# MengLcool/RichSem

Hardware: AMD Instinct MI355X
Metric: training images/sec, RichSem R50 4-scale 1333x800 (MSDeformAttn hot path: 12 fwd + 12 bwd calls per step) (higher is better)
Workload: dtype f32; 1 GPU; configs[1]: R50 4-scale 800x1344 (S=22323), bs=2/GPU, M=8 D=32 L=P=4; per step 6x E(Lq=22323) + 6x Dd(Lq=1092), forward and backward, 12 distinct per-layer tensor sets; loc-init; loc=init, images_per_gpu=2, parallelism=dp1 (replicas, no collective)

## Files before the change

richsem_amd/csrc/msda_rps.h:

```cpp
#pragma once

#include <algorithm>
#include <atomic>
#include <vector>

#include "msda_common.h"

namespace msda {

constexpr int kRpsThreads = 768;
constexpr int kRpsWaves = kRpsThreads / 64;
constexpr int kRpsMaxPx = 312;
constexpr int kRpsMaxSide = 31;
constexpr int kRpsScanThreads = (kRpsMaxPx + 63) / 64 * 64, kRpsScanWaves = kRpsScanThreads / 64;
constexpr int kRpsPpq = (kRpsMaxPx + kRpsThreads / 4 - 1) / (kRpsThreads / 4);
constexpr int kRpsRpl = 2;
constexpr int kRpsChunk = kRpsRpl * kRpsThreads;
constexpr int kRpsSumStride = 36;
constexpr int kRpsSegShift = 3;
constexpr int kRpsMaxSegs = kRpsMaxPx + (kRpsChunk >> kRpsSegShift);
constexpr int kRpsMaxL = 4;
constexpr int kRpsMaxUnits = 448;
constexpr int kRpsD = 32;
constexpr int kRpsPad = 32;
constexpr int kRpsDummyWgs = 2048, kRpsDummyBytes = kRpsDummyWgs * 1024;
constexpr int kRpsMaxRuns = 320;
constexpr int kRpsRunSearch = 256;
static_assert(kRpsRunSearch < kRpsMaxRuns && 2 * kRpsRunSearch >= kRpsMaxRuns, "run search");
constexpr int kRpsQpBits = 19;
constexpr int kRpsPxBits = 9;
static_assert(kRpsMaxPx <= 1 << kRpsPxBits && kRpsQpBits + kRpsPxBits + 4 == 32, "record code: qp | base-grid index | corners");
static_assert(kRpsMaxPx <= kRpsMaxSide * kRpsMaxSide && kRpsScanThreads <= kRpsThreads && kRpsScanWaves * 4 <= 32, "tile grid");
static_assert(kRpsChunk < 1 << 16, "a list's length and a chunk's unit count share a 32-bit word in the scan; slot[] is 16 bits wide");

struct RpsLevel {
    int H, W, start;
    int TH, TW, nty, ntx;
    int bin0;
    int nslab;
    int atomic;
    float inv_TH, inv_TW;
};

struct alignas(16) RpsRec {
    unsigned code;
    float lh, lw, a;
};

struct RpsGeom {
    int N, S, M, Lq, L, P;
    int nunits, ppx;
    int bins_per_pair, nbins;
    RpsLevel lv[kRpsMaxL];
    unsigned units[kRpsMaxUnits];
    unsigned *ctr;
    unsigned long long *bin_state;
    uint2 *runs;
    int max_runs;
    int route_threads;
    unsigned entries_cap;
    struct RpsRec *entries;
    int lut_r[kRpsMaxL], lut_c[kRpsMaxL], lut_n;
    int seg_shift;
    float *dummy;
    unsigned long long *stamps;
};

struct alignas(16) RpsEnt {
    float lh;
    float hwa, lwa;
    unsigned row;
};

struct RpsLds {
    int item_slot[2];
    int wave_tot[16];
    int n_segs, pad[3];
    int uhist[32];
    uint2 runs[kRpsMaxRuns];
    unsigned long long stamp_last, stamp_acc[14];
    int offs[kRpsScanThreads + 4];
    unsigned seg[kRpsMaxSegs + 16];
    RpsEnt ent[kRpsChunk];
    unsigned short slot[kRpsChunk];
    alignas(16) double sum[kRpsMaxPx * kRpsSumStride];
    alignas(16) float vtile[kRpsMaxPx * kRpsD];
};
static_assert(sizeof(RpsLds) <= 160 * 1024, "rps: LDS budget");

__device__ __forceinline__ int rps_wave_scan(int v)
{
    v += __builtin_amdgcn_update_dpp(0, v, 0x111, 0xF, 0xF, true);
    v += __builtin_amdgcn_update_dpp(0, v, 0x112, 0xF, 0xF, true);
    v += __builtin_amdgcn_update_dpp(0, v, 0x114, 0xF, 0xF, true);
    v += __builtin_amdgcn_update_dpp(0, v, 0x118, 0xF, 0xF, true);
    v += __builtin_amdgcn_update_dpp(0, v, 0x142, 0xA, 0xF, false);
    v += __builtin_amdgcn_update_dpp(0, v, 0x143, 0xC, 0xF, false);
    return v;
}

#define RPS_STAMP(i)                                                                   \
    if (kStamps && g.stamps && threadIdx.x == 0) {                                     \
        const unsigned long long now_ = __builtin_amdgcn_s_memtime();                  \
        S->stamp_acc[i] += now_ - S->stamp_last;                                       \
        S->stamp_last = now_;                                                          \
    }

__device__ __forceinline__ unsigned rps_lut_row(const RpsLevel &v, int r)
{
    const int h_low = r - 1, br = max(h_low, 0);
    const int ty = (int)(((float)br + 0.5f) * v.inv_TH);
    const int R0 = ty * v.TH;
    const unsigned gr = (unsigned)(h_low - R0 + 1);
    const unsigned inr = (h_low >= 0 ? 1u : 0u) | (h_low + 1 < v.H ? 2u : 0u);
    return gr | inr << 6 | (unsigned)(ty * v.ntx * v.nslab) << 8;
}
__device__ __forceinline__ unsigned rps_lut_col(const RpsLevel &v, int c)
{
    const int w_low = c - 1, bc = max(w_low, 0);
    const int tx = (int)(((float)bc + 0.5f) * v.inv_TW);
    const int C0 = tx * v.TW, C1 = min(v.W, C0 + v.TW);
    const unsigned gc = (unsigned)(w_low - C0 + 1);
    const unsigned inc = (w_low >= 0 ? 1u : 0u) | (w_low + 1 < v.W ? 2u : 0u);
    const unsigned gw = (unsigned)(C1 - C0 + 1);
    return gc | inc << 6 | (unsigned)(tx * v.nslab) << 8 | gw << 17;
}

constexpr int kRpsRouteThreadsMax = 1024;
static_assert(kRpsMaxUnits <= 512, "route pass: one thread per bin of a pair");

template <int kRpsRouteThreads, int kL = 0, int kP = 0, bool kStamps = false>
__global__ __launch_bounds__(kRpsRouteThreads, 4) void rps_route_kernel(const float *__restrict__ loc, const float *__restrict__ aw,
                                                                     float *__restrict__ grad_value, float *__restrict__ grad_loc,
                                                                     float *__restrict__ grad_aw, const RpsGeom g)
{
    __shared__ unsigned hist[kRpsMaxUnits], base[512];
    __shared__ unsigned wtot[kRpsRouteThreads / kWave];
    __shared__ unsigned sink[kWave];
    extern __shared__ unsigned rps_lut[];
    const int tid = threadIdx.x, lane = tid & (kWave - 1), wave = tid / kWave;
    const int B = g.bins_per_pair;
    const int L = kL ? kL : g.L;
    {
        const int gtid = blockIdx.x * blockDim.x + tid, gsz = gridDim.x * blockDim.x;
        if (gtid < 8) g.ctr[gtid] = 0u;
        if (tid < kWave) sink[tid] = 0u;
        const int row4 = g.M * kRpsD / 4;
        for (int l = 0; l < L; ++l) {
            const RpsLevel &v = g.lv[l];
            for (int i = tid; i <= v.H; i += kRpsRouteThreads) rps_lut[g.lut_r[l] + i] = rps_lut_row(v, i);
            for (int i = tid; i <= v.W; i += kRpsRouteThreads) rps_lut[g.lut_c[l] + i] = rps_lut_col(v, i);
            if (!v.atomic) {
                const int nb = v.nty * v.W + v.ntx * v.H;
                for (int b = 0; b < g.N; ++b) {
                    float4 *dst = reinterpret_cast<float4 *>(grad_value) + (size_t)(b * g.S + v.start) * row4;
                    for (int i = gtid; i < nb * row4; i += gsz) {
                        const int k = i / row4, c = i - k * row4;
                        int px;
                        if (k < v.nty * v.W) {
                            const int ty = k / v.W;
                            px = ty * v.TH * v.W + (k - ty * v.W);
                        } else {
                            const int k2 = k - v.nty * v.W, tx = k2 / v.H;
                            px = (k2 - tx * v.H) * v.W + tx * v.TW;
                        }
                        dst[(size_t)px * row4 + c] = make_float4(0.f, 0.f, 0.f, 0.f);
                    }
                }
                continue;
            }
            const int n4 = v.H * v.W * row4;
            for (int b = 0; b < g.N; ++b) {
                float4 *dst = reinterpret_cast<float4 *>(grad_value) + (size_t)(b * g.S + v.start) * row4;
                for (int i = gtid; i < n4; i += gsz) dst[i] = make_float4(0.f, 0.f, 0.f, 0.f);
            }
        }
    }
    const int P = kP ? kP : g.P, LP = L * P;
    const int qpw = P <= 4 ? 16 : (P <= 8 ? 8 : (P <= 16 ? 4 : (P <= 32 ? 2 : 1)));
    const int ql = lane / P, pp = lane - ql * P;
    const int qpb = qpw * (kRpsRouteThreads / kWave);
    const int qblocks = (g.Lq + qpb - 1) / qpb;
    const int pairs = g.N * g.M;
    const int n_items = pairs * qblocks;
    const unsigned long long lt_mask = (1ull << lane) - 1ull;
    unsigned long long st_acc[8] = {0, 0, 0, 0, 0, 0, 0, 0}, st_last = kStamps && g.stamps ? __builtin_amdgcn_s_memtime() : 0ull;
#define RPS_RSTAMP(i)                                                  \
    if (kStamps && g.stamps) {                                         \
        const unsigned long long now_ = __builtin_amdgcn_s_memtime();  \
        st_acc[i] += now_ - st_last;                                   \
        st_last = now_;                                                \
    }
    float2 xy[kRpsMaxL];
    const int step_pair = (int)(gridDim.x % (unsigned)pairs), step_qb = (int)(gridDim.x / (unsigned)pairs);
    auto item_point = [&](int item_, int pair_, int qb_, bool &live_, int &q_) {
        const int b_ = pair_ / g.M, m_ = pair_ - b_ * g.M;
        q_ = qb_ * qpb + wave * qpw + ql;
        live_ = item_ < n_items && ql < qpw && pp < P && q_ < g.Lq;
        return (unsigned)(((b_ * g.Lq + (live_ ? q_ : 0)) * g.M + m_) * LP + min(pp, P - 1));
    };
    auto request_xy = [&](int item_, int pair_, int qb_) {
        bool live_;
        int q_;
        const unsigned pt0_ = item_point(item_, pair_, qb_, live_, q_);
#pragma unroll
        for (int l = 0; l < kRpsMaxL; ++l) xy[l] = *reinterpret_cast<const float2 *>(loc + 2u * (pt0_ + (unsigned)(min(l, L - 1) * P)));
    };
    int pair = (int)(blockIdx.x % (unsigned)pairs), qb = (int)(blockIdx.x / (unsigned)pairs);
    request_xy(blockIdx.x, pair, qb);
    unsigned long long p_old = 0ull;
    unsigned p_first = 0u, p_cnt = 0u;
    size_t p_gb = 0;
    for (int item = blockIdx.x; item < n_items; item += gridDim.x) {
        for (int i = tid; i < B; i += kRpsRouteThreads) hist[i] = 0u;
        bool live;
        int q;
        const unsigned pt0 = item_point(item, pair, qb, live, q);
        int n_pair = pair + step_pair, n_qb = qb + step_qb;
        if (n_pair >= pairs) {
            n_pair -= pairs;
            ++n_qb;
        }
        n_qb = min(n_qb, qblocks - 1);
        __syncthreads();
        RPS_RSTAMP(1)
        unsigned word[kRpsMaxL];
        unsigned inmap[kRpsMaxL];
        float lh[kRpsMaxL], lw[kRpsMaxL];
        unsigned re[kRpsMaxL], ce[kRpsMaxL];
        unsigned valid_m = 0u, asked_m = 0u, matched_m = 0u;
        unsigned dropped = 0u;
#pragma unroll
        for (int l = 0; l < kRpsMaxL; ++l) {
            lh[l] = lw[l] = 0.f;
            re[l] = ce[l] = 0u;
            if (l >= L) continue;
            const RpsLevel &v = g.lv[l];
            const float Hf = (float)v.H, Wf = (float)v.W;
            const float h_im = xy[l].y * Hf - 0.5f, w_im = xy[l].x * Wf - 0.5f;
            const bool valid = live && h_im > -1.f && w_im > -1.f && h_im < Hf && w_im < Wf;
            valid_m |= valid ? 1u << l : 0u;
            const float hf = floorf(h_im), wf = floorf(w_im);
            lh[l] = h_im - hf;
            lw[l] = w_im - wf;
            dropped |= live && !valid ? 1u << l : 0u;
            re[l] = rps_lut[g.lut_r[l] + (valid ? (int)hf + 1 : 0)];
            ce[l] = rps_lut[g.lut_c[l] + (valid ? (int)wf + 1 : 0)];
        }
        request_xy(item + (int)gridDim.x, n_pair, n_qb);
        float at[kRpsMaxL];
#pragma unroll
        for (int l = 0; l < kRpsMaxL; ++l) at[l] = aw[pt0 + (unsigned)(min(l, L - 1) * P)];
        int ob[kRpsMaxL], lead[kRpsMaxL], lb[kRpsMaxL];
        unsigned own_rank[kRpsMaxL], lt_cnt[kRpsMaxL], n_match[kRpsMaxL];
#pragma unroll
        for (int l = 0; l < kRpsMaxL; ++l) {
            ob[l] = -1;
            lead[l] = 0;
            lb[l] = -1;
            own_rank[l] = lt_cnt[l] = n_match[l] = 0u;
            inmap[l] = 0u;
            word[l] = ~0u;
            if (l >= L) continue;
            const RpsLevel &v = g.lv[l];
            const int ns = v.nslab;
            const int slab = ns > 1 ? uni(qb % ns) : 0;
            ob[l] = (valid_m >> l & 1u) ? v.bin0 + slab + (int)(re[l] >> 8) + (int)((ce[l] >> 8) & 511u) : -1;
            const unsigned inr = (re[l] >> 6) & 3u, inc = (ce[l] >> 6) & 3u;
            inmap[l] = ((inr & 1u) ? inc : 0u) | ((inr & 2u) ? inc << 2 : 0u);
            const unsigned long long vote = __ballot(ob[l] >= 0);
            const int ld = vote ? __ffsll((long long)vote) - 1 : 0;
            lb[l] = __builtin_amdgcn_readlane(ob[l], ld);
            const unsigned long long match = __ballot(ob[l] == lb[l]);
            lead[l] = ld;
            matched_m |= ob[l] == lb[l] && lb[l] >= 0 ? 1u << l : 0u;
            lt_cnt[l] = (unsigned)__popcll(match & lt_mask);
            n_match[l] = (unsigned)__popcll(match);
        }
#pragma unroll
        for (int l = 0; l < kRpsMaxL; ++l) {
            const bool is_lead = lane == lead[l] && lb[l] >= 0, other = ob[l] >= 0 && ob[l] != lb[l];
            const bool asked = is_lead || other;
            asked_m |= asked ? 1u << l : 0u;
            own_rank[l] = atomicAdd(asked ? &hist[is_lead ? lb[l] : ob[l]] : &sink[lane], is_lead ? n_match[l] : (other ? 1u : 0u));
        }
#pragma unroll
        for (int l = 0; l < kRpsMaxL; ++l) {
            if (l >= L) continue;
            const unsigned gr = re[l] & 31u, gc = ce[l] & 31u;
            if (!(asked_m >> l & 1u)) own_rank[l] = lt_cnt[l];
            if (ob[l] >= 0) word[l] = (unsigned)ob[l] | (gr * ((ce[l] >> 17) & 31u) + gc) << 23;
        }
        RPS_RSTAMP(2)
        __syncthreads();
        RPS_RSTAMP(3)
        const unsigned cnt = tid < B ? hist[tid] : 0u;
        const unsigned incl = (unsigned)rps_wave_scan((int)cnt);
        if (lane == kWave - 1) wtot[wave] = incl;
        __syncthreads();
        unsigned before = 0u;
#pragma unroll
        for (int w = 0; w < kRpsRouteThreads / kWave; ++w) before += w < wave ? wtot[w] : 0u;
        const unsigned first = (unsigned)item * (unsigned)(qpb * LP) + before + incl - cnt;
        if (cnt) base[tid] = first;
#pragma unroll
        for (int l = 0; l < kRpsMaxL; ++l) {
            if (l >= L) continue;
            unsigned r = own_rank[l];
            const unsigned rl = (unsigned)__builtin_amdgcn_readlane((int)r, lead[l]);
            if ((matched_m >> l & 1u) && lane != lead[l]) r += rl;
            if (word[l] != ~0u) word[l] |= r << 9;
        }
        __syncthreads();
        RPS_RSTAMP(4)
        const size_t gb = (size_t)pair * B + min(tid, B - 1);
        unsigned long long *const scratch64 = reinterpret_cast<unsigned long long *>(g.dummy + (size_t)(blockIdx.x & (kRpsDummyWgs - 1)) * 256) + lane;
        if (p_cnt) g.runs[p_gb * (size_t)g.max_runs + (size_t)min((unsigned)(p_old >> 32), (unsigned)g.max_runs - 1u)] = make_uint2(p_first, (unsigned)p_old);
        const unsigned long long old = atomicAdd(cnt ? g.bin_state + gb * (kRpsPad / 2) : scratch64, cnt ? (1ull << 32) | (unsigned long long)cnt : 0ull);
        const unsigned qp = (unsigned)((live ? q : 0) * P + pp);
        unsigned slot0[kRpsMaxL];
#pragma unroll
        for (int l = 0; l < kRpsMaxL; ++l) slot0[l] = base[word[l] & 511u];
        asm volatile("" : "+v"(at[0]), "+v"(at[1]), "+v"(at[2]), "+v"(at[3]));
#pragma unroll
        for (int l = 0; l < kRpsMaxL; ++l) {
            const unsigned w = word[l];
            if (w != ~0u) {
                const unsigned slot = min(slot0[l] + ((w >> 9) & 16383u), g.entries_cap - 1u);
                const unsigned code = qp | (w >> 23) << kRpsQpBits | inmap[l] << (kRpsQpBits + kRpsPxBits);
                g.entries[slot] = RpsRec{code, lh[l], lw[l], at[l]};
            }
        }
        if (__ballot(dropped != 0u)) {
#pragma unroll
            for (int l = 0; l < kRpsMaxL; ++l)
                if (dropped >> l & 1u) {
                    const unsigned pt = pt0 + (unsigned)(l * P);
                    grad_aw[pt] = 0.f;
                    *reinterpret_cast<float2 *>(grad_loc + 2u * pt) = make_float2(0.f, 0.f);
                }
        }
        RPS_RSTAMP(5)
        p_old = old;
        p_first = first;
        p_cnt = cnt;
        p_gb = gb;
        pair = n_pair;
        qb = n_qb;
        RPS_RSTAMP(6)
        __syncthreads();
        RPS_RSTAMP(7)
    }
    if (p_cnt) g.runs[p_gb * (size_t)g.max_runs + (size_t)min((unsigned)(p_old >> 32), (unsigned)g.max_runs - 1u)] = make_uint2(p_first, (unsigned)p_old);
    if (kStamps && g.stamps && tid == 0)
        for (int i = 0; i < 8; ++i) g.stamps[(size_t)(1024 + blockIdx.x) * 16 + i] = st_acc[i];
#undef RPS_RSTAMP
}

typedef float rps_v2f __attribute__((ext_vector_type(2)));
typedef float rps_v4f __attribute__((ext_vector_type(4)));

__device__ __forceinline__ float rps_quad_rotated_sum(float x0, float x1, float x2, float x3)
{
    const float ra = x0 + dpp_f<kDppXor1>(x1);
    const float rb = x2 + dpp_f<kDppXor1>(x3);
    return ra + dpp_f<kDppXor2>(rb);
}

template <typename TV>
struct RpsRow;
template <>
struct RpsRow<float> {
    float4 a, b;
    __device__ __forceinline__ void load(const float *base, unsigned off)
    {
        a = *reinterpret_cast<const float4 *>(reinterpret_cast<const char *>(base) + off);
        b = *reinterpret_cast<const float4 *>(reinterpret_cast<const char *>(base) + off + 64u);
    }
    __device__ __forceinline__ void unpack(rps_v2f (&gq)[4]) const
    {
        gq[0] = (rps_v2f){a.x, a.y}; gq[1] = (rps_v2f){a.z, a.w};
        gq[2] = (rps_v2f){b.x, b.y}; gq[3] = (rps_v2f){b.z, b.w};
    }
};
template <>
struct RpsRow<bf16_t> {
    uint2 a, b;
    __device__ __forceinline__ void load(const bf16_t *base, unsigned off)
    {
        a = *reinterpret_cast<const uint2 *>(reinterpret_cast<const char *>(base) + off);
        b = *reinterpret_cast<const uint2 *>(reinterpret_cast<const char *>(base) + off + 32u);
    }
    __device__ __forceinline__ void unpack(rps_v2f (&gq)[4]) const
    {
        gq[0] = (rps_v2f){__uint_as_float(a.x << 16), __uint_as_float(a.x & 0xFFFF0000u)};
        gq[1] = (rps_v2f){__uint_as_float(a.y << 16), __uint_as_float(a.y & 0xFFFF0000u)};
        gq[2] = (rps_v2f){__uint_as_float(b.x << 16), __uint_as_float(b.x & 0xFFFF0000u)};
        gq[3] = (rps_v2f){__uint_as_float(b.y << 16), __uint_as_float(b.y & 0xFFFF0000u)};
    }
};

template <bool P4, typename TV = float, bool kStamps = false>
__global__ __launch_bounds__(kRpsThreads, kRpsThreads / 256) void rps_tile_kernel(
    const TV *__restrict__ value, const TV *__restrict__ grad_out, TV *__restrict__ grad_value, float *__restrict__ grad_acc,
    float *__restrict__ grad_loc, float *__restrict__ grad_aw, const RpsGeom g)
{
    extern __shared__ __attribute__((aligned(16))) unsigned char smem[];
    RpsLds *S = reinterpret_cast<RpsLds *>(smem);

    const int tid = threadIdx.x, lane = tid & (kWave - 1), wave = tid / kWave;
    const int j4 = tid & 3, quad = tid >> 2;
    const int c_lo = 4 * j4, c_hi = 16 + 4 * j4;
    const float w_ys = (j4 & 2) ? 1.f : -1.f, w_yc = (j4 & 2) ? 0.f : 1.f;
    const unsigned w_xoff = (j4 & 1) ? 8u : 4u;
    const unsigned lane_row = (unsigned)(c_lo * sizeof(TV));
    const int P = P4 ? 4 : g.P;
    const int LP = g.L * P;
    const int row_elems = g.M * kRpsD;
    const int pairs = g.N * g.M;
    const int xq = blockIdx.x & (kXcds - 1);
    const int n_items = g.nunits * g.ppx;
    float *const dummy_w = g.dummy + (size_t)(blockIdx.x & (kRpsDummyWgs - 1)) * 256;
    if (kStamps && g.stamps && tid == 0) {
        for (int i = 0; i < 14; ++i) S->stamp_acc[i] = 0;
        S->stamp_last = __builtin_amdgcn_s_memtime();
    }
    struct Item {
        bool live;
        int l, b, m, H, W, R0, R1, C0, C1, gw, npx;
    };
    auto item_geom = [&](int id) {
        Item it;
        const unsigned unit = (unsigned)uni((int)g.units[min(id, n_items - 1) / g.ppx]);
        const int pr = xq + kXcds * (min(id, n_items - 1) % g.ppx);
        const int pair = min(pr, pairs - 1);
        it.live = id < n_items && pr < pairs;
        it.l = unit & 3;
        const int ty = (unit >> 2) & 63, tx = (unit >> 8) & 63;
        it.b = pair / g.M;
        it.m = pair - it.b * g.M;
        it.H = g.lv[it.l].H;
        it.W = g.lv[it.l].W;
        it.R0 = ty * g.lv[it.l].TH;
        it.R1 = min(it.H, it.R0 + g.lv[it.l].TH);
        it.C0 = tx * g.lv[it.l].TW;
        it.C1 = min(it.W, it.C0 + g.lv[it.l].TW);
        it.gw = it.C1 - it.C0 + 1;
        it.npx = it.live ? (it.R1 - it.R0 + 1) * it.gw : 0;
        return it;
    };
    auto bin_range_raw = [&](int id, unsigned &bin_, unsigned &okm_, unsigned long long &st_) {
        const int idc = min(id, n_items - 1);
        const unsigned unit = g.units[idc / g.ppx];
        const int pair = xq + kXcds * (idc % g.ppx);
        const bool ok = id < n_items && pair < pairs;
        const int l = unit & 3, ty = (unit >> 2) & 63, tx = (unit >> 8) & 63, slab = (unit >> 14) & 255, nslab = (unit >> 22) & 255;
        const unsigned bin_c = ok ? (unsigned)(pair * g.bins_per_pair + g.lv[l].bin0 + (ty * g.lv[l].ntx + tx) * nslab + slab) : 0u;
        st_ = g.bin_state[(size_t)bin_c * (kRpsPad / 2)];
        okm_ = ok ? 0xFFFFFFFFu : 0u;
        bin_ = bin_c | ~okm_;
    };
    auto bin_counts = [&](unsigned long long st_, unsigned okm_, int &n, int &nr) {
        unsigned lo = (unsigned)st_, hi = (unsigned)(st_ >> 32);
        asm volatile("" : "+v"(lo), "+v"(hi));
        n = (int)(min(lo, 0x7FFFFFFFu) & okm_);
        nr = (int)(min(hi, (unsigned)min(g.max_runs, kRpsMaxRuns)) & okm_);
    };
    auto bin_range = [&](int id, unsigned &bin_, int &n, int &nr) {
        const int idc = min(id, n_items - 1);
        const unsigned unit = g.units[idc / g.ppx];
        const int pair = xq + kXcds * (idc % g.ppx);
        const bool ok = id < n_items && pair < pairs;
        const int l = unit & 3, ty = (unit >> 2) & 63, tx = (unit >> 8) & 63, slab = (unit >> 14) & 255, nslab = (unit >> 22) & 255;
        const unsigned bin_c = ok ? (unsigned)(pair * g.bins_per_pair + g.lv[l].bin0 + (ty * g.lv[l].ntx + tx) * nslab + slab) : 0u;
        const unsigned long long st = g.bin_state[(size_t)bin_c * (kRpsPad / 2)];
        const unsigned okm = ok ? 0xFFFFFFFFu : 0u;
        bin_ = bin_c | ~okm;
        n = (int)(min((unsigned)st, 0x7FFFFFFFu) & okm);
        nr = (int)(min((unsigned)(st >> 32), (unsigned)min(g.max_runs, kRpsMaxRuns)) & okm);
    };
    uint2 run_reg = make_uint2(0u, 0u);
    auto load_runs = [&](unsigned bin_, int nr) {
        const int i = min(tid, max(uni(nr) - 1, 0));
        const unsigned b_ = (unsigned)uni((int)bin_);
        run_reg = g.runs[(size_t)(b_ == 0xFFFFFFFFu ? 0u : b_) * g.max_runs + i];
    };
    auto park_runs = [&]() {
        if (tid < kRpsMaxRuns) S->runs[tid] = run_reg;
    };
    RpsRec n_rec[kRpsRpl];
    unsigned n_idx[kRpsRpl];
    auto fetch_recs = [&](int n_, int nr_, int ch) {
        const int n = uni(n_), nr = uni(nr_);
        const int T = max((nr + kWave - 1) / kWave, 1);
        const bool s_ok = lane * T < nr;
        const unsigned sy = S->runs[min(lane * T, max(nr - 1, 0))].y;
        const int k_last = max(n - 1, 0);
#pragma unroll
        for (int u = 0; u < kRpsRpl; ++u) {
            const int kb = ch * kRpsChunk + u * kRpsThreads + wave * kWave;
            const unsigned k = (unsigned)min(kb + lane, k_last);
            const unsigned k_lo = (unsigned)min(kb, k_last), k_hi = (unsigned)min(kb + kWave - 1, k_last);
            const int c_lo = __popcll(__ballot(s_ok && sy <= k_lo)) - 1, c_hi = __popcll(__ballot(s_ok && sy <= k_hi)) - 1;
            const int ra = max(c_lo, 0) * T, rb = min((max(c_hi, 0) + 1) * T, nr);
            int r = ra;
            for (int step = rb - ra > 1 ? 1 << (31 - __builtin_clz(rb - ra - 1)) : 0; step > 0; step >>= 1) {
                const int cand = r + step;
                if (cand < rb && S->runs[cand].y <= k) r = cand;
            }
            const uint2 run = S->runs[r];
            n_idx[u] = n > 0 ? min(run.x + (k - run.y), g.entries_cap - 1u) : 0u;
            n_rec[u] = g.entries[n_idx[u]];
        }
    };
    float4 nv[kRpsPpq][2];
    auto fetch_rows = [&](const Item &it) {
#pragma unroll
        for (int r = 0; r < kRpsPpq; ++r) {
            const int px = min(quad + r * (kRpsThreads / 4), max(it.npx - 1, 0));
            const int gr_ = px / it.gw, gc_ = px - gr_ * it.gw;
            const int prow_ = min(it.R0 + gr_, it.H - 1), pcol_ = min(it.C0 + gc_, it.W - 1);
            const TV *src = value + ((int64_t)(it.b * g.S + g.lv[it.l].start + prow_ * it.W + pcol_) * g.M + it.m) * kRpsD;
            nv[r][0] = ld4(src + c_lo);
            nv[r][1] = ld4(src + c_hi);
        }
    };
    auto store_rows = [&]() {
#pragma unroll
        for (int r = 0; r < kRpsPpq; ++r) {
            const int px = quad + r * (kRpsThreads / 4);
            if (px < kRpsMaxPx) {
                *reinterpret_cast<float4 *>(S->vtile + px * kRpsD + c_lo) = nv[r][0];
                *reinterpret_cast<float4 *>(S->vtile + px * kRpsD + c_hi) = nv[r][1];
            }
        }
    };

    unsigned *const draw_at = tid == 0 ? g.ctr + xq : reinterpret_cast<unsigned *>(dummy_w) + (tid & 255);
    const unsigned draw_by = tid == 0 ? 1u : 0u;
    unsigned draw = atomicAdd(draw_at, draw_by);
    if (tid == 0) S->item_slot[0] = (int)draw;
    draw = atomicAdd(draw_at, draw_by);
    __syncthreads();
    int item_id = uni(S->item_slot[0]);
    unsigned e_bin;
    int n_ent, n_runs;
    bin_range(item_id, e_bin, n_ent, n_runs);
    e_bin = (unsigned)uni((int)e_bin);
    n_ent = uni(n_ent);
    n_runs = uni(n_runs);
    load_runs(e_bin, n_runs);
    park_runs();
    __syncthreads();
    fetch_recs(n_ent, n_runs, 0);
    Item it = item_geom(item_id);
    int par = 0;
    fetch_rows(it);
    for (int i = tid; i < kRpsMaxPx * kRpsSumStride / 2; i += kRpsThreads) reinterpret_cast<double2 *>(S->sum)[i] = make_double2(0.0, 0.0);

    while (item_id < n_items) {
        if (tid == 0) S->item_slot[par ^ 1] = (int)draw;
        const int l = it.l, b = it.b, m = it.m, H = it.H, W = it.W, R0 = it.R0, R1 = it.R1, C0 = it.C0, C1 = it.C1, gw = it.gw;
        const int npx = it.npx;
        const int n_chunks = it.live ? (n_ent + kRpsChunk - 1) / kRpsChunk : 0;
        const int bq0 = b * g.Lq;
        float *const vt = S->vtile;
        __syncthreads();
        const int next_id = uni(S->item_slot[par ^ 1]);
        unsigned next_bin, next_ok;
        unsigned long long next_st;
        int next_n = 0, next_runs = 0;
        bin_range_raw(next_id, next_bin, next_ok, next_st);
        const Item nit = item_geom(next_id);
        store_rows();
        RPS_STAMP(0)

        for (int ch = 0; ch < n_chunks; ++ch) {
            const int n_here = min(kRpsChunk, n_ent - ch * kRpsChunk);
            for (int i = tid; i <= npx; i += kRpsThreads) S->offs[i] = 0;
            int pbase[kRpsRpl], pos[kRpsRpl];
#pragma unroll
            for (int u = 0; u < kRpsRpl; ++u) pos[u] = -1;
            if (ch == 0) draw = atomicAdd(draw_at, draw_by);
            __syncthreads();
            RPS_STAMP(1)
#pragma unroll
            for (int u = 0; u < kRpsRpl; ++u) {
                pbase[u] = min((int)((n_rec[u].code >> kRpsQpBits) & ((1u << kRpsPxBits) - 1u)), kRpsMaxPx - 1);
                if (u * kRpsThreads + tid < n_here) pos[u] = atomicAdd(&S->offs[pbase[u]], 1);
            }
            __syncthreads();
            RPS_STAMP(2)

            {
                const int sh = g.seg_shift;
                int c = 0, v = 0, incl = 0, n_full = 0, part = 0, pslot = 0, n0 = 0, incl0 = 0, rank = 0, mycnt = 0;
                if (tid < kRpsScanThreads) {
                    c = tid < npx ? S->offs[tid] : 0;
                    v = c | ((c + (1 << sh) - 1) >> sh) << 16;
                    n_full = c >> sh;
                    part = c & ((1 << sh) - 1);
                    pslot = part ? 3 - ((part - 1) >> (sh - 2)) : -1;
                    n0 = n_full + (pslot == 0 ? 1 : 0);
                    incl = rps_wave_scan(v);
                    incl0 = rps_wave_scan(n0);
                    if (lane == kWave - 1) S->wave_tot[wave] = incl;
                    mycnt = __builtin_amdgcn_readlane(incl0, kWave - 1);
                    const unsigned long long lt = (1ull << lane) - 1ull;
#pragma unroll
                    for (int k = 1; k < 4; ++k) {
                        const unsigned long long bk = __ballot(pslot == k);
                        if (pslot == k) rank = __popcll(bk & lt);
                        if (lane == k) mycnt = __popcll(bk);
                    }
                    if (lane < 4) S->uhist[wave * 4 + lane] = mycnt;
                }
                __syncthreads();
                if (tid < kRpsScanThreads) {
                    int base = 0;
#pragma unroll
                    for (int w = 0; w < kRpsScanWaves; ++w) base += w < wave ? S->wave_tot[w] : 0;
                    const int excl = base + incl - v;
                    if (tid <= npx) S->offs[tid] = excl & 0xFFFF;
                    if (tid == kRpsScanThreads - 1) {
                        if (npx == kRpsScanThreads) S->offs[npx] = (base + incl) & 0xFFFF;
                        S->n_segs = (base + incl) >> 16;
                    }
                    int sbk[4], run_ = 0;
#pragma unroll
                    for (int k = 0; k < 4; ++k) {
                        int tot = 0, mine_before = 0;
#pragma unroll
                        for (int w = 0; w < kRpsScanWaves; ++w) {
                            const int x = S->uhist[w * 4 + k];
                            tot += x;
                            mine_before += w < wave ? x : 0;
                        }
                        sbk[k] = run_ + mine_before;
                        run_ += tot;
                    }
                    const int at0 = sbk[0] + incl0 - n0;
                    const int atp = (pslot == 1 ? sbk[1] : (pslot == 2 ? sbk[2] : sbk[3])) + rank;
                    for (int sgm = 0; sgm < n_full; ++sgm) S->seg[at0 + sgm] = (unsigned)(tid | sgm << 16);
                    if (pslot == 0) S->seg[at0 + n_full] = (unsigned)(tid | n_full << 16);
                    else if (pslot > 0) S->seg[atp] = (unsigned)(tid | n_full << 16);
                }
            }
            __syncthreads();
            RPS_STAMP(3)

#pragma unroll
            for (int u = 0; u < kRpsRpl; ++u)
                if (pos[u] >= 0) {
                    const int e = pos[u] + S->offs[pbase[u]];
                    const unsigned qp = n_rec[u].code & ((1u << kRpsQpBits) - 1u);
                    const int q = P4 ? (int)(qp >> 2) : (int)(qp / (unsigned)P);
                    const float lwa = n_rec[u].lw * n_rec[u].a;
                    S->ent[e] = RpsEnt{n_rec[u].lh, (1.f - n_rec[u].lw) * n_rec[u].a, lwa, (unsigned)((bq0 + q) * g.M + m) * (unsigned)(kRpsD * sizeof(TV))};
                    S->slot[u * kRpsThreads + tid] = (unsigned short)e;
                }
            __syncthreads();
            RPS_STAMP(4)

            const int n_segs = uni(S->n_segs);
            for (int u0 = wave * 16; u0 < n_segs; u0 += kRpsWaves * 16) {
                unsigned long long wt0 = 0, wt1 = 0, wt2 = 0;
                if (kStamps && g.stamps && tid == 0) wt0 = __builtin_amdgcn_s_memtime();
                const int un = u0 + (lane >> 2);
                if (un < n_segs) {
                    const unsigned sc = S->seg[un];
                    const int my_p = (int)(sc & 0xFFFFu);
                    int e = S->offs[my_p] + (int)((sc >> 16) << g.seg_shift);
                    const int e1 = min(e + (1 << g.seg_shift), S->offs[my_p + 1]);
                    const int lr = my_p / gw, lc = my_p - lr * gw;
                    const int r0 = max(lr - 1, 0) * gw, c0 = max(lc - 1, 0);
                    rps_v2f v[4][4];
                    {
                        const int row_hi = lr * gw - r0, col_hi = lc - c0;
                        const int row_same = (j4 & 2) ? row_hi : 0, row_flip = row_hi - row_same;
                        const int col_same = (j4 & 1) ? col_hi : 0, col_flip = col_hi - col_same;
                        const float *const v00 = vt + (r0 + c0) * kRpsD;
#pragma unroll
                        for (int r = 0; r < 4; ++r) {
                            const float *const src = v00 + (((r & 2) ? row_flip : row_same) + ((r & 1) ? col_flip : col_same)) * kRpsD;
                            const float4 a0 = *reinterpret_cast<const float4 *>(src + c_lo);
                            const float4 a1 = *reinterpret_cast<const float4 *>(src + c_hi);
                            v[r][0] = (rps_v2f){a0.x, a0.y}; v[r][1] = (rps_v2f){a0.z, a0.w};
                            v[r][2] = (rps_v2f){a1.x, a1.y}; v[r][3] = (rps_v2f){a1.z, a1.w};
                        }
                    }
                    rps_v4f macc[8];
#pragma unroll
                    for (int m_ = 0; m_ < 8; ++m_) macc[m_] = (rps_v4f){0.f, 0.f, 0.f, 0.f};
#define RPS_POINT(ROW, CF, EP)                                                                                                   \
    {                                                                                                                            \
        const float wj = __builtin_fmaf(w_ys, CF.x, w_yc) * CF.y;                                                                \
        rps_v2f gq[4];                                                                                                           \
        ROW.unpack(gq);                                                                                                          \
        _Pragma("unroll") for (int c = 0; c < 4; ++c)                                                                            \
        {                                                                                                                        \
            macc[2 * c] = __builtin_amdgcn_mfma_f32_4x4x1f32(wj, gq[c].x, macc[2 * c], 0, 0, 0);                                 \
            macc[2 * c + 1] = __builtin_amdgcn_mfma_f32_4x4x1f32(wj, gq[c].y, macc[2 * c + 1], 0, 0, 0);                         \
        }                                                                                                                        \
        float d[4];                                                                                                              \
        _Pragma("unroll") for (int k = 0; k < 4; ++k)                                                                            \
        {                                                                                                                        \
            rps_v2f t = gq[0] * v[k][0];                                                                                         \
            t += gq[1] * v[k][1];                                                                                                \
            t += gq[2] * v[k][2];                                                                                                \
            t += gq[3] * v[k][3];                                                                                                \
            d[k] = t.x + t.y;                                                     \
        }                                                                                                                        \
                                               \
        *RPS_LDS(float, (EP) + 4u * (unsigned)j4) = rps_quad_rotated_sum(d[0], d[1], d[2], d[3]);                                \
    }
#define RPS_ROW(OFF, ROW) ROW.load(grad_out, (OFF) + lane_row);
#define RPS_OFF(EP) (*RPS_LDS(const unsigned, (EP) + 12u))
#define RPS_LDS(T, A) (reinterpret_cast<__attribute__((address_space(3))) T *>((size_t)(A)))
                    unsigned ent_lds = (unsigned)(size_t)(__attribute__((address_space(3))) char *)(S->ent);
                    asm volatile("" : "+v"(ent_lds));
                    unsigned ep = ent_lds + (unsigned)e * 16u;
                    const unsigned ep_end = ent_lds + (unsigned)e1 * 16u, ep_last = ep_end - 16u;
                    if (kStamps && g.stamps && wave == 0) {
                        int len = e1 - e;
                        for (int o = 32; o > 0; o >>= 1) len = max(len, __shfl_xor(len, o));
                        if (tid == 0) S->stamp_acc[13] += (unsigned long long)len;
                    }
#define RPS_CF(EP) make_float2(*RPS_LDS(const float, EP), *RPS_LDS(const float, (EP) + w_xoff))
                    unsigned offA = RPS_OFF(ep), offB = RPS_OFF(min(ep + 16u, ep_last));
                    float2 cA = RPS_CF(ep), cB = RPS_CF(min(ep + 16u, ep_last));
                    RpsRow<TV> gA, gB;
                    RPS_ROW(offA, gA)
                    if (kStamps && g.stamps && tid == 0) wt1 = __builtin_amdgcn_s_memtime();
                    for (; ep + 16u < ep_end; ep += 32u) {
                        RPS_ROW(offB, gB)
                        const unsigned nA = min(ep + 32u, ep_last), nB = min(ep + 48u, ep_last);
                        offA = RPS_OFF(nA);
                        const float2 cA2 = RPS_CF(nA);
                        RPS_POINT(gA, cA, ep)
                        RPS_ROW(offA, gA)
                        offB = RPS_OFF(nB);
                        const float2 cB2 = RPS_CF(nB);
                        RPS_POINT(gB, cB, ep + 16u)
                        cA = cA2;
                        cB = cB2;
                    }
                    if (ep < ep_end) RPS_POINT(gA, cA, ep)
#undef RPS_CF
#undef RPS_LDS
#undef RPS_OFF
#undef RPS_ROW
#undef RPS_POINT
                    if (kStamps && g.stamps && tid == 0) wt2 = __builtin_amdgcn_s_memtime();
#pragma unroll
                    for (int k = 0; k < 4; ++k) {
                        const bool ok = (k >= 2 || lr >= 1) && ((k & 1) || lc >= 1);
                        if (ok) {
                            double *dst = S->sum + (my_p - (k < 2 ? gw : 0) - ((k & 1) ? 0 : 1)) * kRpsSumStride + j4;
#pragma unroll
                            for (int m_ = 0; m_ < 8; ++m_) atomicAdd(dst + 4 * m_, (double)macc[m_][k]);
                        }
                    }
                }
                if (kStamps && g.stamps && tid == 0 && wt1) {
                    const unsigned long long wt3 = __builtin_amdgcn_s_memtime();
                    S->stamp_acc[9] += wt1 - wt0;
                    S->stamp_acc[10] += wt2 - wt1;
                    S->stamp_acc[11] += wt3 - wt2;
                    S->stamp_acc[12] += 1;
                }
            }
            RpsRec c_rec[kRpsRpl];
#pragma unroll
            for (int u = 0; u < kRpsRpl; ++u) {
                unsigned ix = n_idx[u];
                asm volatile("" : "+v"(ix));
                c_rec[u] = g.entries[ix];
            }
            const bool last_chunk = ch + 1 == n_chunks;
            bin_counts(next_st, next_ok, next_n, next_runs);
            load_runs(next_bin, next_runs);
            fetch_recs(n_ent, n_runs, min(ch + 1, n_chunks - 1));
            __syncthreads();
            if (last_chunk) park_runs();
            RPS_STAMP(5)

            float ga_[kRpsRpl], gx_[kRpsRpl], gy_[kRpsRpl];
            unsigned pt_[kRpsRpl];
            bool mine_[kRpsRpl];
#pragma unroll
            for (int u = 0; u < kRpsRpl; ++u) {
                const int k = min(u * kRpsThreads + tid, n_here - 1);
                const RpsRec r = c_rec[u];
                float4 d = *reinterpret_cast<const float4 *>(S->ent + S->slot[k]);
                const unsigned in = r.code >> (kRpsQpBits + kRpsPxBits);
                if (!(in & 1u)) d.x = 0.f;
                if (!(in & 2u)) d.y = 0.f;
                if (!(in & 4u)) d.z = 0.f;
                if (!(in & 8u)) d.w = 0.f;
                const float lh = r.lh, lw = r.lw, hh = 1.f - lh, hw = 1.f - lw;
                const float s_a = hh * hw * d.x + hh * lw * d.y + lh * hw * d.z + lh * lw * d.w;
                const float s_w = hh * (d.y - d.x) + lh * (d.w - d.z);
                const float s_h = hw * (d.z - d.x) + lw * (d.w - d.y);
                const unsigned qp = r.code & ((1u << kRpsQpBits) - 1u);
                const unsigned q = P4 ? qp >> 2 : qp / (unsigned)P, pp = qp - q * (unsigned)P;
                pt_[u] = (unsigned)((bq0 + (int)q) * g.M + m) * (unsigned)LP + (unsigned)(l * P) + pp;
                mine_[u] = u * kRpsThreads + tid < n_here;
                ga_[u] = s_a;
                gx_[u] = (float)W * s_w * r.a;
                gy_[u] = (float)H * s_h * r.a;
            }
#pragma unroll
            for (int u = 0; u < kRpsRpl; ++u) {
                *(mine_[u] ? grad_aw + pt_[u] : dummy_w + lane) = ga_[u];
                *(mine_[u] ? reinterpret_cast<float2 *>(grad_loc + 2u * pt_[u]) : reinterpret_cast<float2 *>(dummy_w) + lane) = make_float2(gx_[u], gy_[u]);
            }
            RPS_STAMP(6)
        }
        if (n_chunks == 0) {
            draw = atomicAdd(draw_at, draw_by);
            bin_counts(next_st, next_ok, next_n, next_runs);
            load_runs(next_bin, next_runs);
            __syncthreads();
            park_runs();
        }
        fetch_rows(nit);
        __syncthreads();
        fetch_recs(next_n, next_runs, 0);
        if (tid == 0 && e_bin != 0xFFFFFFFFu) g.bin_state[(size_t)e_bin * (kRpsPad / 2)] = 0ull;
        if (!g.lv[l].atomic) {
#pragma unroll
            for (int r = 0; r < kRpsPpq; ++r) {
                const int px = quad + r * (kRpsThreads / 4);
                const int pxc = min(px, kRpsMaxPx - 1);
                const int gr = pxc / gw, gc = pxc - gr * gw;
                const int prow = R0 + gr, pcol = C0 + gc;
                const bool interior = px < npx && gr >= 1 && gc >= 1 && prow < R1 && pcol < C1;
                double *src = S->sum + pxc * kRpsSumStride + j4;
                const int64_t px_off = ((int64_t)(b * g.S + g.lv[l].start + prow * W + pcol) * g.M + m) * kRpsD;
                TV *const dst = interior ? grad_value + px_off : reinterpret_cast<TV *>(dummy_w) + 4 * lane - c_lo;
                st4(dst + c_lo, make_float4((float)src[0], (float)src[4], (float)src[8], (float)src[12]));
                st4(interior ? dst + c_hi : dst + c_lo, make_float4((float)src[16], (float)src[20], (float)src[24], (float)src[28]));
                if (interior) {
#pragma unroll
                    for (int k = 0; k < 8; ++k) src[4 * k] = 0.0;
                }
            }
            const int c32 = tid & 31;
            const int64_t tile_base = ((int64_t)(b * g.S + g.lv[l].start) * g.M + m) * kRpsD + c32;
            const int gh = R1 - R0 + 1, n_border = npx ? 2 * (gw + gh) - 4 : 0;
            for (int k = tid >> 5; k < n_border; k += kRpsThreads / 32) {
                const int k2 = k - 2 * gw;
                const int pr = k < gw ? 0 : (k2 < 0 ? gh - 1 : 1 + (k2 >> 1));
                const int pc = k < gw ? k : (k2 < 0 ? k - gw : ((k2 & 1) ? gw - 1 : 0));
                const int row = R0 + pr, col = C0 + pc;
                double *const sp = S->sum + (pr * gw + pc) * kRpsSumStride + (c32 & 16) + 4 * (c32 & 3) + ((c32 & 15) >> 2);
                const float x = (float)*sp;
                *sp = 0.0;
                if (row < H && col < W && x != 0.f) atomicAdd(grad_acc + tile_base + (int64_t)(row * W + col) * row_elems, x);
            }
        } else if (n_chunks > 0) {
            const int c32 = tid & 31;
            const int64_t tile_base = ((int64_t)(b * g.S + g.lv[l].start) * g.M + m) * kRpsD + c32;
            for (int p = tid >> 5; p < npx; p += kRpsThreads / 32) {
                const int pr = p / gw, row = R0 + pr, col = C0 + (p - pr * gw);
                double *const sp = S->sum + p * kRpsSumStride + (c32 & 16) + 4 * (c32 & 3) + ((c32 & 15) >> 2);
                const float x = (float)*sp;
                *sp = 0.0;
                if (row < H && col < W && x != 0.f) atomicAdd(grad_acc + tile_base + (int64_t)(row * W + col) * row_elems, x);
            }
        }
        __syncthreads();
        RPS_STAMP(7)
        item_id = next_id;
        e_bin = (unsigned)uni((int)next_bin);
        n_ent = uni(next_n);
        n_runs = uni(next_runs);
        it = nit;
        par ^= 1;
    }
    if (kStamps && g.stamps && tid == 0) {
        const unsigned long long now_ = __builtin_amdgcn_s_memtime();
        S->stamp_acc[8] += now_ - S->stamp_last;
        for (int i = 0; i < 14; ++i) g.stamps[(size_t)blockIdx.x * 16 + i] = S->stamp_acc[i];
    }
}

__global__ __launch_bounds__(256) void rps_round_kernel(const float *__restrict__ acc, bf16_t *__restrict__ grad_value, const RpsGeom g)
{
    const int gtid = blockIdx.x * blockDim.x + threadIdx.x, gsz = gridDim.x * blockDim.x;
    const int row4 = g.M * kRpsD / 4;
    for (int l = 0; l < g.L; ++l) {
        const RpsLevel &v = g.lv[l];
        const int nb = v.nty * v.W + v.ntx * v.H;
        const int n4 = (v.atomic ? v.H * v.W : nb) * row4;
        for (int b = 0; b < g.N; ++b) {
            const size_t base = (size_t)(b * g.S + v.start) * row4 * 4;
            for (int i = gtid; i < n4; i += gsz) {
                size_t at = (size_t)i;
                if (!v.atomic) {
                    const int k = i / row4, c = i - k * row4;
                    int px;
                    if (k < v.nty * v.W) {
                        const int ty = k / v.W;
                        px = ty * v.TH * v.W + (k - ty * v.W);
                    } else {
                        const int k2 = k - v.nty * v.W, tx = k2 / v.H;
                        px = (k2 - tx * v.H) * v.W + tx * v.TW;
                    }
                    at = (size_t)px * row4 + c;
                }
                st4(grad_value + base + 4 * at, *reinterpret_cast<const float4 *>(acc + base + 4 * at));
            }
        }
    }
}

struct RpsOptions {
    std::atomic<int> tile{16};
    std::atomic<int> max_chunks{12};
    std::atomic<int> route_wgs{2};
    std::atomic<int> order{0};
    std::atomic<int> seg_shift{4};
};
inline RpsOptions &rps_options()
{
    static RpsOptions o;
    return o;
}

struct RpsPlan {
    bool ok = false;
    RpsGeom g{};
    size_t max_entries = 0;
};

inline RpsPlan plan_rps(int N, int S, int M, int D, int L, int Lq, int P, const int64_t *shapes, const int64_t *lsi)
{
    RpsPlan pl;
    if (D != kRpsD || L < 1 || L > kRpsMaxL || P < 1 || P > 64) return pl;
    int64_t pre = 0;
    bool tiles_s = true;
    for (int l = 0; l < L; ++l) {
        tiles_s = tiles_s && lsi[l] == pre;
        pre += shapes[2 * l] * shapes[2 * l + 1];
        if (shapes[2 * l] >= 32768 || shapes[2 * l + 1] >= 32768) return pl;
    }
    if (!tiles_s || pre != S) return pl;
    const int64_t n_pts = (int64_t)N * Lq * M * L * P;
    if (n_pts >= ((int64_t)1 << 30) || (int64_t)Lq * P >= ((int64_t)1 << kRpsQpBits)) return pl;
    RpsGeom &g = pl.g;
    g.N = N; g.S = S; g.M = M; g.Lq = Lq; g.L = L; g.P = P;
    g.seg_shift = std::max(kRpsSegShift, std::min(11, rps_options().seg_shift.load()));
    g.ppx = (N * M + kXcds - 1) / kXcds;
    const int tile_opt = rps_options().tile.load();
    const int tmax = tile_opt >= 16 ? kRpsMaxSide - 1 : std::max(1, tile_opt - 1), max_chunks = std::max(1, rps_options().max_chunks.load());
    struct U { unsigned code; int64_t cost; };
    std::vector<U> units;
    int bins = 0;
    for (int l = 0; l < L; ++l) {
        RpsLevel &v = g.lv[l];
        v.H = (int)shapes[2 * l]; v.W = (int)shapes[2 * l + 1]; v.start = (int)lsi[l];
        const double per_px = (double)Lq * P / ((double)v.H * v.W);
        auto chunks_of = [&](int th, int tw) { return (int)(per_px * th * tw * 1.05 / kRpsChunk) + 1; };
        auto slabs_of = [&](int nchunks) { return std::min(255, std::max(1, (nchunks + max_chunks - 1) / max_chunks)); };
        int64_t best = -1;
        v.TH = v.TW = v.nty = v.ntx = 0;
        for (int nty = 1; nty <= std::min(64, v.H); ++nty) {
            const int th = (v.H + nty - 1) / nty;
            if (th > tmax || (v.H + th - 1) / th != nty) continue;
            int tried = 0;
            for (int ntx = 1; ntx <= std::min(64, v.W) && tried < 4; ++ntx) {
                const int tw = (v.W + ntx - 1) / ntx;
                if (tw > tmax || (th + 1) * (tw + 1) > kRpsMaxPx || (v.W + tw - 1) / tw != ntx) continue;
                ++tried;
                const int nch = chunks_of(th, tw);
                const int64_t cost = (int64_t)nty * ntx * (5 * slabs_of(nch) + 2 * nch);
                if (best < 0 || cost < best) {
                    best = cost;
                    v.TH = th; v.TW = tw; v.nty = nty; v.ntx = ntx;
                }
            }
        }
        if (best < 0) return pl;
        const int nchunks = chunks_of(v.TH, v.TW);
        v.nslab = slabs_of(nchunks);
        v.atomic = v.nslab > 1 ? 1 : 0;
        v.inv_TH = 1.0f / (float)v.TH;
        v.inv_TW = 1.0f / (float)v.TW;
        v.bin0 = bins;
        bins += v.nty * v.ntx * v.nslab;
        for (int ty = 0; ty < v.nty; ++ty)
            for (int tx = 0; tx < v.ntx; ++tx)
                for (int sl = 0; sl < v.nslab; ++sl)
                    units.push_back(U{(unsigned)l | (unsigned)ty << 2 | (unsigned)tx << 8 | (unsigned)sl << 14 | (unsigned)v.nslab << 22,
                                      (int64_t)(nchunks + v.nslab - 1) / v.nslab * 16 + 8});
    }
    if (units.size() > (size_t)kRpsMaxUnits) return pl;
    g.lut_n = 0;
    for (int l = 0; l < L; ++l) {
        g.lut_r[l] = g.lut_n;
        g.lut_n += g.lv[l].H + 1;
        g.lut_c[l] = g.lut_n;
        g.lut_n += g.lv[l].W + 1;
    }
    if (g.lut_n > kRpsMaxL * 2 * 962) return pl;
    if (rps_options().order.load() == 0) {
        std::stable_sort(units.begin(), units.end(), [](const U &a, const U &b) { return a.cost > b.cost; });
    } else {
        std::vector<int> order;
        for (int l = 0; l < L; ++l)
            if (g.lv[l].nslab == 1) order.push_back(l);
        std::sort(order.begin(), order.end(), [&](int a, int b) { return g.lv[a].nty * g.lv[a].ntx < g.lv[b].nty * g.lv[b].ntx; });
        auto key_of = [&](unsigned code) {
            const int l = code & 3, ty = (code >> 2) & 63, tx = (code >> 8) & 63, nslab = (code >> 22) & 255;
            if (nslab > 1) return (unsigned long long)0;
            const RpsLevel &v = g.lv[l];
            const double cy = (std::min(v.H, ty * v.TH + v.TH) + ty * v.TH) * 0.5 / v.H, cx = (std::min(v.W, tx * v.TW + v.TW) + tx * v.TW) * 0.5 / v.W;
            unsigned long long key = 1ull << 60;
            int shift = 42;
            for (int k : order) {
                const RpsLevel &u = g.lv[k];
                unsigned long long part = 0;
                if (u.nty * u.ntx <= v.nty * v.ntx || k == l) {
                    const int uy = k == l ? ty : std::min(u.nty - 1, (int)(cy * u.H / u.TH)), ux = k == l ? tx : std::min(u.ntx - 1, (int)(cx * u.W / u.TW));
                    part = (unsigned long long)((uy + 1) << 7 | (ux + 1));
                }
                key |= part << shift;
                shift -= 14;
                if (k == l) break;
            }
            return key;
        };
        std::stable_sort(units.begin(), units.end(), [&](const U &a, const U &b) {
            const unsigned long long ka = key_of(a.code), kb = key_of(b.code);
            return ka != kb ? ka < kb : a.cost > b.cost;
        });
    }
    g.nunits = (int)units.size();
    for (int i = 0; i < g.nunits; ++i) g.units[i] = units[i].code;
    g.bins_per_pair = bins;
    g.nbins = bins * N * M;
    const int qpw = P <= 4 ? 16 : (P <= 8 ? 8 : (P <= 16 ? 4 : (P <= 32 ? 2 : 1)));
    g.route_threads = 512;
    g.max_runs = (Lq + qpw * 8 - 1) / (qpw * 8);
    if (g.max_runs > kRpsMaxRuns) {
        g.route_threads = kRpsRouteThreadsMax;
        g.max_runs = (Lq + qpw * 16 - 1) / (qpw * 16);
    }
    if (g.max_runs > kRpsMaxRuns) return pl;
    const int qpb = qpw * (g.route_threads / kWave);
    pl.max_entries = (size_t)N * M * g.max_runs * (size_t)qpb * L * P;
    if (pl.max_entries >= ((size_t)1 << 32)) return pl;
    pl.ok = true;
    return pl;
}

}
```

Before: 741.0 img/s.

## Pipeline next-next item lookahead and move tile stores across item boundary in RPS backward

Restructures the persistent RPS backward loop so that the item after next is drawn and its bin state read one iteration early. The shared-memory tile store for the next item now happens at the end of the current iteration instead of after a barrier at the top of the loop, which removes one __syncthreads per item. Entry records are loaded as raw uint4 vectors, and asm volatile register pins are added to steer when the compiler issues loads. The cost is more live registers and more complex control flow (the ahead flag for empty items), which could lower occupancy or introduce ordering bugs.

After: 741.0 img/s, median of 3. No clear change (+0.0%).

```diff
diff --git a/richsem_amd/csrc/msda_rps.h b/richsem_amd/csrc/msda_rps.h
--- a/richsem_amd/csrc/msda_rps.h
+++ b/richsem_amd/csrc/msda_rps.h
@@ -359,6 +359,14 @@
 
 typedef float rps_v2f __attribute__((ext_vector_type(2)));
 typedef float rps_v4f __attribute__((ext_vector_type(4)));
+typedef unsigned rps_v4u __attribute__((ext_vector_type(4)));
+
+__device__ __forceinline__ RpsRec rps_rec_of(const rps_v4u &r) { return RpsRec{r.x, __uint_as_float(r.y), __uint_as_float(r.z), __uint_as_float(r.w)}; }
+__device__ __forceinline__ RpsRec rps_rec_take(rps_v4u &r)
+{
+    asm volatile("" : "+v"(r));
+    return rps_rec_of(r);
+}
 
 __device__ __forceinline__ float rps_quad_rotated_sum(float x0, float x1, float x2, float x3)
 {
@@ -486,9 +494,10 @@
         run_reg = g.runs[(size_t)(b_ == 0xFFFFFFFFu ? 0u : b_) * g.max_runs + i];
     };
     auto park_runs = [&]() {
+        asm volatile("" : "+v"(run_reg.x), "+v"(run_reg.y));
         if (tid < kRpsMaxRuns) S->runs[tid] = run_reg;
     };
-    RpsRec n_rec[kRpsRpl];
+    rps_v4u n_rec[kRpsRpl];
     unsigned n_idx[kRpsRpl];
     auto fetch_recs = [&](int n_, int nr_, int ch) {
         const int n = uni(n_), nr = uni(nr_);
@@ -510,7 +519,7 @@
             }
             const uint2 run = S->runs[r];
             n_idx[u] = n > 0 ? min(run.x + (k - run.y), g.entries_cap - 1u) : 0u;
-            n_rec[u] = g.entries[n_idx[u]];
+            n_rec[u] = *reinterpret_cast<const rps_v4u *>(g.entries + n_idx[u]);
         }
     };
     float4 nv[kRpsPpq][2];
@@ -527,6 +536,8 @@
     };
     auto store_rows = [&]() {
 #pragma unroll
+        for (int r = 0; r < kRpsPpq; ++r) asm volatile("" : : "v"(nv[r][0].x), "v"(nv[r][1].x));
+#pragma unroll
         for (int r = 0; r < kRpsPpq; ++r) {
             const int px = quad + r * (kRpsThreads / 4);
             if (px < kRpsMaxPx) {
@@ -541,6 +552,7 @@
     unsigned draw = atomicAdd(draw_at, draw_by);
     if (tid == 0) S->item_slot[0] = (int)draw;
     draw = atomicAdd(draw_at, draw_by);
+    if (tid == 0) S->item_slot[1] = (int)draw;
     __syncthreads();
     int item_id = uni(S->item_slot[0]);
     unsigned e_bin;
@@ -551,28 +563,28 @@
     n_runs = uni(n_runs);
     load_runs(e_bin, n_runs);
     park_runs();
+    int next_id = uni(S->item_slot[1]);
+    unsigned next_bin, next_ok;
+    unsigned long long next_st;
+    int next_n = 0, next_runs = 0;
+    bin_range_raw(next_id, next_bin, next_ok, next_st);
+    Item nit = item_geom(next_id);
     __syncthreads();
     fetch_recs(n_ent, n_runs, 0);
     Item it = item_geom(item_id);
     int par = 0;
+    bool ahead = false;
     fetch_rows(it);
     for (int i = tid; i < kRpsMaxPx * kRpsSumStride / 2; i += kRpsThreads) reinterpret_cast<double2 *>(S->sum)[i] = make_double2(0.0, 0.0);
+    store_rows();
+    __syncthreads();
 
     while (item_id < n_items) {
-        if (tid == 0) S->item_slot[par ^ 1] = (int)draw;
         const int l = it.l, b = it.b, m = it.m, H = it.H, W = it.W, R0 = it.R0, R1 = it.R1, C0 = it.C0, C1 = it.C1, gw = it.gw;
         const int npx = it.npx;
         const int n_chunks = it.live ? (n_ent + kRpsChunk - 1) / kRpsChunk : 0;
         const int bq0 = b * g.Lq;
         float *const vt = S->vtile;
-        __syncthreads();
-        const int next_id = uni(S->item_slot[par ^ 1]);
-        unsigned next_bin, next_ok;
-        unsigned long long next_st;
-        int next_n = 0, next_runs = 0;
-        bin_range_raw(next_id, next_bin, next_ok, next_st);
-        const Item nit = item_geom(next_id);
-        store_rows();
         RPS_STAMP(0)
 
         for (int ch = 0; ch < n_chunks; ++ch) {
@@ -584,9 +596,11 @@
             if (ch == 0) draw = atomicAdd(draw_at, draw_by);
             __syncthreads();
             RPS_STAMP(1)
+            RpsRec rec[kRpsRpl];
 #pragma unroll
             for (int u = 0; u < kRpsRpl; ++u) {
-                pbase[u] = min((int)((n_rec[u].code >> kRpsQpBits) & ((1u << kRpsPxBits) - 1u)), kRpsMaxPx - 1);
+                rec[u] = rps_rec_of(n_rec[u]);
+                pbase[u] = min((int)((rec[u].code >> kRpsQpBits) & ((1u << kRpsPxBits) - 1u)), kRpsMaxPx - 1);
                 if (u * kRpsThreads + tid < n_here) pos[u] = atomicAdd(&S->offs[pbase[u]], 1);
             }
             __syncthreads();
@@ -653,10 +667,10 @@
             for (int u = 0; u < kRpsRpl; ++u)
                 if (pos[u] >= 0) {
                     const int e = pos[u] + S->offs[pbase[u]];
-                    const unsigned qp = n_rec[u].code & ((1u << kRpsQpBits) - 1u);
+                    const unsigned qp = rec[u].code & ((1u << kRpsQpBits) - 1u);
                     const int q = P4 ? (int)(qp >> 2) : (int)(qp / (unsigned)P);
-                    const float lwa = n_rec[u].lw * n_rec[u].a;
-                    S->ent[e] = RpsEnt{n_rec[u].lh, (1.f - n_rec[u].lw) * n_rec[u].a, lwa, (unsigned)((bq0 + q) * g.M + m) * (unsigned)(kRpsD * sizeof(TV))};
+                    const float lwa = rec[u].lw * rec[u].a;
+                    S->ent[e] = RpsEnt{rec[u].lh, (1.f - rec[u].lw) * rec[u].a, lwa, (unsigned)((bq0 + q) * g.M + m) * (unsigned)(kRpsD * sizeof(TV))};
                     S->slot[u * kRpsThreads + tid] = (unsigned short)e;
                 }
             __syncthreads();
@@ -770,12 +784,12 @@
                     S->stamp_acc[12] += 1;
                 }
             }
-            RpsRec c_rec[kRpsRpl];
+            rps_v4u c_rec[kRpsRpl];
 #pragma unroll
             for (int u = 0; u < kRpsRpl; ++u) {
                 unsigned ix = n_idx[u];
                 asm volatile("" : "+v"(ix));
-                c_rec[u] = g.entries[ix];
+                c_rec[u] = *reinterpret_cast<const rps_v4u *>(g.entries + ix);
             }
             const bool last_chunk = ch + 1 == n_chunks;
             bin_counts(next_st, next_ok, next_n, next_runs);
@@ -791,7 +805,7 @@
 #pragma unroll
             for (int u = 0; u < kRpsRpl; ++u) {
                 const int k = min(u * kRpsThreads + tid, n_here - 1);
-                const RpsRec r = c_rec[u];
+                const RpsRec r = rps_rec_take(c_rec[u]);
                 float4 d = *reinterpret_cast<const float4 *>(S->ent + S->slot[k]);
                 const unsigned in = r.code >> (kRpsQpBits + kRpsPxBits);
                 if (!(in & 1u)) d.x = 0.f;
@@ -815,27 +829,47 @@
                 *(mine_[u] ? grad_aw + pt_[u] : dummy_w + lane) = ga_[u];
                 *(mine_[u] ? reinterpret_cast<float2 *>(grad_loc + 2u * pt_[u]) : reinterpret_cast<float2 *>(dummy_w) + lane) = make_float2(gx_[u], gy_[u]);
             }
+#pragma unroll
+            for (int u = 0; u < kRpsRpl; ++u) asm volatile("" : "+v"(n_rec[u]));
             RPS_STAMP(6)
         }
         if (n_chunks == 0) {
-            draw = atomicAdd(draw_at, draw_by);
-            bin_counts(next_st, next_ok, next_n, next_runs);
-            load_runs(next_bin, next_runs);
-            __syncthreads();
-            park_runs();
-        }
+            if (!ahead) {
+                draw = atomicAdd(draw_at, draw_by);
+                bin_counts(next_st, next_ok, next_n, next_runs);
+                load_runs(next_bin, next_runs);
+                park_runs();
+            } else {
+                park_runs();
+            }
+        }
+        asm volatile("" : "+v"(draw));
+        if (tid == 0) S->item_slot[par] = (int)draw;
+        const bool next_empty = !nit.live || uni(next_n) == 0;
         fetch_rows(nit);
         __syncthreads();
+        const int nn_id = uni(S->item_slot[par]);
+        unsigned nn_bin, nn_ok;
+        unsigned long long nn_st;
+        bin_range_raw(nn_id, nn_bin, nn_ok, nn_st);
+        const Item nnit = item_geom(nn_id);
+        int nn_n = 0, nn_runs = 0;
+        if (next_empty) {
+            draw = atomicAdd(draw_at, draw_by);
+            bin_counts(nn_st, nn_ok, nn_n, nn_runs);
+            asm volatile("" : "+v"(draw));
+            load_runs(nn_bin, nn_runs);
+        }
         fetch_recs(next_n, next_runs, 0);
-        if (tid == 0 && e_bin != 0xFFFFFFFFu) g.bin_state[(size_t)e_bin * (kRpsPad / 2)] = 0ull;
-        if (!g.lv[l].atomic) {
+        const bool shared_tile = g.lv[l].atomic != 0;
+        {
 #pragma unroll
             for (int r = 0; r < kRpsPpq; ++r) {
                 const int px = quad + r * (kRpsThreads / 4);
                 const int pxc = min(px, kRpsMaxPx - 1);
                 const int gr = pxc / gw, gc = pxc - gr * gw;
                 const int prow = R0 + gr, pcol = C0 + gc;
-                const bool interior = px < npx && gr >= 1 && gc >= 1 && prow < R1 && pcol < C1;
+                const bool interior = !shared_tile && px < npx && gr >= 1 && gc >= 1 && prow < R1 && pcol < C1;
                 double *src = S->sum + pxc * kRpsSumStride + j4;
                 const int64_t px_off = ((int64_t)(b * g.S + g.lv[l].start + prow * W + pcol) * g.M + m) * kRpsD;
                 TV *const dst = interior ? grad_value + px_off : reinterpret_cast<TV *>(dummy_w) + 4 * lane - c_lo;
@@ -846,6 +880,13 @@
                     for (int k = 0; k < 8; ++k) src[4 * k] = 0.0;
                 }
             }
+        }
+        store_rows();
+#pragma unroll
+        for (int u = 0; u < kRpsRpl; ++u) asm volatile("" : "+v"(n_rec[u]));
+        asm volatile("" : "+v"(run_reg.x), "+v"(run_reg.y));
+        if (tid == 0 && e_bin != 0xFFFFFFFFu) g.bin_state[(size_t)e_bin * (kRpsPad / 2)] = 0ull;
+        if (!shared_tile) {
             const int c32 = tid & 31;
             const int64_t tile_base = ((int64_t)(b * g.S + g.lv[l].start) * g.M + m) * kRpsD + c32;
             const int gh = R1 - R0 + 1, n_border = npx ? 2 * (gw + gh) - 4 : 0;
@@ -877,6 +918,14 @@
         n_ent = uni(next_n);
         n_runs = uni(next_runs);
         it = nit;
+        next_id = nn_id;
+        next_bin = nn_bin;
+        next_ok = nn_ok;
+        next_st = nn_st;
+        next_n = nn_n;
+        next_runs = nn_runs;
+        ahead = next_empty;
+        nit = nnit;
         par ^= 1;
     }
     if (kStamps && g.stamps && tid == 0) {
```
